# UMEssen/Body-and-Organ-Analysis

Hardware: AMD Instinct MI355X
Metric: CT volumes/sec (512^3 @1.5 mm, total+bca) on MI355X (higher is better)
Workload: dtype f16

## Files before the change

### body-and-organ-analysis_amd/csrc/ccl_bits.hip

```cpp
#include <string.h>

#include <algorithm>

#include "common.h"
#include "ccl_tile.h"

#define CB_CAP 1024
#define CB_BG 0xFFFFu

struct CbGeom {
    int Z, Y, X, W;
    int tx, ty, tz;
    size_t words;
    size_t vox;
    size_t tiles;
};

__host__ __device__ __forceinline__ unsigned cb_valid_word(int X, int w) {
    const int left = X - 32 * w;
    return left >= 32 ? 0xFFFFFFFFu : (left <= 0 ? 0u : ((1u << left) - 1u));
}

struct CbLut {
    unsigned char v[256];
};

__global__ __launch_bounds__(256) void k_bits_select(const unsigned char* __restrict__ seg, CbGeom g, CbLut lut, int n_masks, unsigned* __restrict__ bits) {
    __shared__ unsigned char s_lut[256];
    s_lut[threadIdx.x] = lut.v[threadIdx.x];
    __syncthreads();
    const size_t wi = (size_t)blockIdx.x * 256 + threadIdx.x;
    if (wi >= g.words) return;
    const int w = (int)(wi % g.W);
    const size_t row = wi / g.W;
    const unsigned char* p = seg + row * g.X + (size_t)w * 32;
    const int cnt = min(32, g.X - w * 32);
    unsigned out[8] = {0, 0, 0, 0, 0, 0, 0, 0};
    if (cnt == 32 && (((uintptr_t)p) & 15) == 0) {
        const uint4 a = *(const uint4*)p, b = *(const uint4*)(p + 16);
        const unsigned ww[8] = {a.x, a.y, a.z, a.w, b.x, b.y, b.z, b.w};
#pragma unroll
        for (int k = 0; k < 8; ++k)
#pragma unroll
            for (int j = 0; j < 4; ++j) {
                const unsigned m = s_lut[(ww[k] >> (8 * j)) & 0xFFu];
#pragma unroll
                for (int q = 0; q < 8; ++q) out[q] |= ((m >> q) & 1u) << (4 * k + j);
            }
    } else {
        for (int i = 0; i < cnt; ++i) {
            const unsigned m = s_lut[p[i]];
#pragma unroll
            for (int q = 0; q < 8; ++q) out[q] |= ((m >> q) & 1u) << i;
        }
    }
#pragma unroll
    for (int q = 0; q < 8; ++q)
        if (q < n_masks) bits[(size_t)q * g.words + wi] = out[q];
}

__global__ __launch_bounds__(256) void k_bits_unpack(const unsigned* __restrict__ bits, CbGeom g, unsigned char* __restrict__ out) {
    const size_t wi = (size_t)blockIdx.x * 256 + threadIdx.x;
    if (wi >= g.words) return;
    const int w = (int)(wi % g.W);
    const size_t row = wi / g.W;
    const unsigned v = bits[wi];
    unsigned char* p = out + row * g.X + (size_t)w * 32;
    const int cnt = min(32, g.X - w * 32);
    if (cnt == 32 && (((uintptr_t)p) & 15) == 0) {
        unsigned ww[8];
#pragma unroll
        for (int k = 0; k < 8; ++k) {
            const unsigned n4 = (v >> (4 * k)) & 0xfu;
            ww[k] = (n4 & 1u) | ((n4 & 2u) << 7) | ((n4 & 4u) << 14) | ((n4 & 8u) << 21);
        }
        *(uint4*)p = make_uint4(ww[0], ww[1], ww[2], ww[3]);
        *(uint4*)(p + 16) = make_uint4(ww[4], ww[5], ww[6], ww[7]);
    } else {
        for (int i = 0; i < cnt; ++i) p[i] = (unsigned char)((v >> i) & 1u);
    }
}

__global__ __launch_bounds__(256) void k_bits_erode_axis(const unsigned* __restrict__ in, CbGeom g, int axis, int lo, int hi, unsigned* __restrict__ out) {
    const size_t wi = (size_t)blockIdx.x * 256 + threadIdx.x;
    if (wi >= g.words) return;
    const int w = (int)(wi % g.W);
    const size_t row = wi / g.W;
    const int y = (int)(row % g.Y), z = (int)(row / g.Y);
    unsigned r = 0xFFFFFFFFu;
    if (axis == 2) {
        auto word = [&](int ww) -> unsigned {
            if (ww < 0 || ww >= g.W) return 0xFFFFFFFFu;
            return in[row * g.W + ww] | ~cb_valid_word(g.X, ww);
        };
        const unsigned prev = word(w - 1), cur = word(w), next = word(w + 1);
        for (int d = lo; d <= hi; ++d) {
            unsigned v;
            if (d == 0)
                v = cur;
            else if (d < 0)
                v = (cur << (-d)) | (prev >> (32 + d));
            else
                v = (cur >> d) | (next << (32 - d));
            r &= v;
        }
    } else {
        const int pos = axis == 0 ? z : y, len = axis == 0 ? g.Z : g.Y;
        const long long st = axis == 0 ? (long long)g.Y * g.W : (long long)g.W;
        for (int d = lo; d <= hi; ++d) {
            const int q = pos + d;
            if (q < 0 || q >= len) continue;
            r &= in[(long long)wi + d * st];
        }
    }
    out[wi] = r & cb_valid_word(g.X, w);
}

struct CbLabels {
    unsigned char v[8];
};
__global__ __launch_bounds__(256) void k_bits_assign(const unsigned* __restrict__ bits, CbGeom g, int n_masks, CbLabels labels, unsigned char* __restrict__ out) {
    const size_t wi = (size_t)blockIdx.x * 256 + threadIdx.x;
    if (wi >= g.words) return;
    const int w = (int)(wi % g.W);
    const size_t row = wi / g.W;
    unsigned m[8];
#pragma unroll
    for (int q = 0; q < 8; ++q) m[q] = q < n_masks ? bits[(size_t)q * g.words + wi] : 0u;
    unsigned char* p = out + row * g.X + (size_t)w * 32;
    const int cnt = min(32, g.X - w * 32);
    unsigned any = 0;
#pragma unroll
    for (int q = 0; q < 8; ++q) any |= m[q];
    if (!any) return;
    unsigned char b[32];
#pragma unroll
    for (int i = 0; i < 32; ++i) {
        unsigned char v = 0;
#pragma unroll
        for (int q = 0; q < 8; ++q)
            if ((m[q] >> i) & 1u) v = labels.v[q];
        b[i] = v;
    }
    if (cnt == 32 && (((uintptr_t)p) & 15) == 0) {
        const uint4 o0 = *(const uint4*)p, o1 = *(const uint4*)(p + 16);
        const unsigned oo[8] = {o0.x, o0.y, o0.z, o0.w, o1.x, o1.y, o1.z, o1.w};
        unsigned ww[8];
#pragma unroll
        for (int k = 0; k < 8; ++k) {
            unsigned v = 0;
#pragma unroll
            for (int j = 0; j < 4; ++j) {
                const unsigned keep = (oo[k] >> (8 * j)) & 0xFFu;
                v |= (((any >> (4 * k + j)) & 1u) ? (unsigned)b[4 * k + j] : keep) << (8 * j);
            }
            ww[k] = v;
        }
        *(uint4*)p = make_uint4(ww[0], ww[1], ww[2], ww[3]);
        *(uint4*)(p + 16) = make_uint4(ww[4], ww[5], ww[6], ww[7]);
    } else {
        for (int i = 0; i < cnt; ++i)
            if ((any >> i) & 1u) p[i] = b[i];
    }
}

__host__ __device__ inline int cb_fill_stride(int W) { return W | 1; }

__global__ __launch_bounds__(256) void k_bits_fill2d(const unsigned* __restrict__ in, CbGeom g, unsigned* __restrict__ out) {
    extern __shared__ unsigned int fsm2[];
    const int Y = g.Y, W = g.W, X = g.X;
    const int WP = cb_fill_stride(W);
    unsigned int* bg = fsm2;
    unsigned int* rc = fsm2 + (size_t)Y * WP;
    __shared__ int changed;
    const int tid = threadIdx.x;
    const size_t base = (size_t)blockIdx.y * g.words + (size_t)blockIdx.x * Y * W;
    const int nw = Y * W;
    for (int idx = tid; idx < nw; idx += 256) {
        const int y = idx / W, w = idx - y * W;
        const unsigned b = ~in[base + idx] & cb_valid_word(X, w);
        unsigned r = 0;
        if (y == 0 || y == Y - 1) r = b;
        if (w == 0) r |= b & 1u;
        if (w == W - 1) r |= b & (1u << ((X - 1) & 31));
        bg[y * WP + w] = b;
        rc[y * WP + w] = r;
    }
    __syncthreads();
    for (;;) {
        if (tid == 0) changed = 0;
        __syncthreads();
        int ch = 0;
        for (int y = tid; y < Y; y += 256) {
            unsigned int* rr = rc + y * WP;
            const unsigned int* bb = bg + y * WP;
            unsigned int carry = 0;
            for (int w = 0; w < W; ++w) {
                const unsigned int b = bb[w];
                unsigned int sd = rr[w] | (carry ? (b & 1u) : 0u);
                const unsigned long long sum = (unsigned long long)b + sd;
                const unsigned int nr = sd | ((b ^ (unsigned int)sum) & b);
                carry = (unsigned int)(sum >> 32);
                if (nr != rr[w]) { rr[w] = nr; ch = 1; }
            }
            carry = 0;
            for (int w = W - 1; w >= 0; --w) {
                const unsigned int b = __brev(bb[w]);
                unsigned int sd = __brev(rr[w]) | (carry ? (b & 1u) : 0u);
                const unsigned long long sum = (unsigned long long)b + sd;
                const unsigned int nr = __brev(sd | ((b ^ (unsigned int)sum) & b));
                carry = (unsigned int)(sum >> 32);
                if (nr != rr[w]) { rr[w] = nr; ch = 1; }
            }
        }
        __syncthreads();
        for (int idx = tid; idx < nw; idx += 256) {
            const int y = idx / W, li = idx + y * (WP - W);
            const unsigned int r = rc[li];
            const unsigned int up = y > 0 ? rc[li - WP] : 0u, dn = y < Y - 1 ? rc[li + WP] : 0u;
            const unsigned int nr = r | ((up | dn) & bg[li]);
            if (nr != r) { rc[li] = nr; ch = 1; }
        }
        if (ch) changed = 1;
        __syncthreads();
        if (!changed) break;
        __syncthreads();
    }
    for (int idx = tid; idx < nw; idx += 256) {
        const int y = idx / W, w = idx - y * W, li = y * WP + w;
        out[base + idx] = (~bg[li] | (bg[li] & ~rc[li])) & cb_valid_word(X, w);
    }
}

struct CbTab {
    int* parent;
    unsigned* size;
    int* first;
    int* ncomp;
    unsigned short* ids;
};

__device__ __forceinline__ unsigned cb_word(const unsigned* __restrict__ bits, const CbGeom& g, int m, int z, int y, int w, int inv) {
    if (z < 0 || y < 0 || w < 0 || z >= g.Z || y >= g.Y || w >= g.W) return 0u;
    const unsigned v = bits[(size_t)m * g.words + ((size_t)z * g.Y + y) * g.W + w];
    return inv ? (~v & cb_valid_word(g.X, w)) : v;
}

__global__ __launch_bounds__(256) void k_cb_local(const unsigned* __restrict__ bits, CbGeom g, int inv, CbTab T) {
    __shared__ int lab[CCL_TILE];
    __shared__ unsigned int rowbits[CCL_TY * CCL_TZ];
    __shared__ unsigned int rootbits[CCL_TY * CCL_TZ];
    __shared__ int rowpre[CCL_TY * CCL_TZ + 1];
    const int tid = threadIdx.x, m = blockIdx.y;
    int t = blockIdx.x;
    const int tx = t % g.tx;
    t /= g.tx;
    const int ty = t % g.ty, tz = t / g.ty;
    const int x0 = tx * CCL_TX, y0 = ty * CCL_TY, z0 = tz * CCL_TZ;
    const size_t tile = (size_t)m * g.tiles + blockIdx.x;
    {
        const int ly = tid % CCL_TY, lz = tid / CCL_TY;
        rowbits[tid] = cb_word(bits, g, m, z0 + lz, y0 + ly, tx, inv);
    }
    __syncthreads();
    {
        const unsigned w = rowbits[tid];
        const int all0 = __syncthreads_and(w == 0u);
        const int all1 = __syncthreads_and(w == 0xffffffffu);
        if (all0) {
            if (tid == 0) T.ncomp[tile] = 0;
            return;
        }
        if (all1) {
            if (tid == 0) {
                const int gid = (int)(blockIdx.x) * CB_CAP;
                const size_t e = (size_t)m * g.tiles * CB_CAP + gid;
                T.ncomp[tile] = -1;
                T.parent[e] = gid;
                T.size[e] = CCL_TILE;
                T.first[e] = (int)(((size_t)z0 * g.Y + y0) * g.X + x0);
            }
            return;
        }
    }
    ccl_tile_init_runs(rowbits, lab, tid);
    __syncthreads();
    ccl_tile_union_rows(rowbits, lab, tid);
    __syncthreads();
    int myroot[CCL_TILE / 256];
    ccl_tile_roots(rowbits, lab, tid, myroot);
    __syncthreads();
#pragma unroll
    for (int k = 0; k < CCL_TILE / 256; ++k) {
        const int r2 = (tid >> 5) + 8 * k, lx = tid & 31;
        const unsigned long long b = __ballot(myroot[k] == r2 * CCL_TX + lx);
        if (lx == 0) rootbits[r2] = (unsigned int)(b >> (32 * ((tid >> 5) & 1)));
    }
    unsigned int* cnt = (unsigned int*)lab;
#pragma unroll
    for (int k = 0; k < CCL_TILE / 256; ++k) cnt[tid + 256 * k] = 0;
    __syncthreads();
    {
        const int c = __popc(rootbits[tid]);
        int s = c;
#pragma unroll
        for (int d = 1; d < 64; d <<= 1) {
            const int o = __shfl_up(s, d);
            if ((tid & 63) >= d) s += o;
        }
        __shared__ int wtot[4];
        if ((tid & 63) == 63) wtot[tid >> 6] = s;
        __syncthreads();
        int basew = 0;
        for (int w = 0; w < (tid >> 6); ++w) basew += wtot[w];
        rowpre[tid] = basew + s - c;
        if (tid == 255) rowpre[256] = basew + s;
    }
    ccl_tile_count_runs(cnt, tid, myroot);
    __syncthreads();
    const int n_local = rowpre[256];
    int did[CCL_TILE / 256];
#pragma unroll
    for (int k = 0; k < CCL_TILE / 256; ++k) {
        const int r2 = (tid >> 5) + 8 * k, lx = tid & 31;
        did[k] = -1;
        if (myroot[k] == r2 * CCL_TX + lx) {
            const int d = rowpre[r2] + __popc(rootbits[r2] & ((1u << lx) - 1u));
            did[k] = d;
            const int gid = (int)blockIdx.x * CB_CAP + d;
            const size_t e = (size_t)m * g.tiles * CB_CAP + gid;
            const int ly = r2 % CCL_TY, lz = r2 / CCL_TY;
            T.parent[e] = gid;
            T.size[e] = cnt[r2 * CCL_TX + lx];
            T.first[e] = (int)(((size_t)(z0 + lz) * g.Y + (y0 + ly)) * g.X + (x0 + lx));
        }
    }
    __syncthreads();
#pragma unroll
    for (int k = 0; k < CCL_TILE / 256; ++k)
        if (did[k] >= 0) lab[((tid >> 5) + 8 * k) * CCL_TX + (tid & 31)] = did[k];
    if (tid == 0) T.ncomp[tile] = n_local;
    __syncthreads();
#pragma unroll
    for (int k = 0; k < CCL_TILE / 256; ++k) {
        const int r2 = (tid >> 5) + 8 * k, lx = tid & 31, ly = r2 % CCL_TY, lz = r2 / CCL_TY;
        const int x = x0 + lx, y = y0 + ly, z = z0 + lz;
        if (x >= g.X || y >= g.Y || z >= g.Z) continue;
        T.ids[(size_t)m * g.vox + ((size_t)z * g.Y + y) * g.X + x] = myroot[k] >= 0 ? (unsigned short)lab[myroot[k]] : (unsigned short)CB_BG;
    }
}

__device__ __forceinline__ int cb_gid(const CbGeom& g, const CbTab& T, int m, int x, int y, int z) {
    const int tile = ((z / CCL_TZ) * g.ty + (y / CCL_TY)) * g.tx + (x / CCL_TX);
    const int nc = T.ncomp[(size_t)m * g.tiles + tile];
    if (nc < 0) return tile * CB_CAP;
    return tile * CB_CAP + (int)T.ids[(size_t)m * g.vox + ((size_t)z * g.Y + y) * g.X + x];
}

__device__ __forceinline__ void cb_border_voxel(const unsigned* __restrict__ bits, const CbGeom& g, const CbTab& T, int m, int inv, int x, int y, int z) {
    const int lx = x % CCL_TX, ly = y % CCL_TY, lz = z % CCL_TZ;
    const int w = x >> 5;
    const unsigned me = cb_word(bits, g, m, z, y, w, inv);
    if (!((me >> lx) & 1u)) return;
    int* P = T.parent + (size_t)m * g.tiles * CB_CAP;
    int my = -1;
    auto mine = [&]() {
        if (my < 0) my = cb_gid(g, T, m, x, y, z);
        return my;
    };
    const bool me_full = T.ncomp[(size_t)m * g.tiles + ((z / CCL_TZ) * g.ty + (y / CCL_TY)) * g.tx + (x / CCL_TX)] < 0;
    auto link = [&](int xx, int yy, int zz) {
        if (me_full && T.ncomp[(size_t)m * g.tiles + ((zz / CCL_TZ) * g.ty + (yy / CCL_TY)) * g.tx + (xx / CCL_TX)] < 0) return;
        uf_union(P, mine(), cb_gid(g, T, m, xx, yy, zz));
    };
    auto row3 = [&](int yy, int zz, bool& b0, bool& b1, bool& b2) {
        const unsigned wc = cb_word(bits, g, m, zz, yy, w, inv);
        b1 = (wc >> lx) & 1u;
        b0 = lx > 0 ? ((wc >> (lx - 1)) & 1u) : (x > 0 && (cb_word(bits, g, m, zz, yy, w - 1, inv) >> 31));
        b2 = lx < 31 ? ((wc >> (lx + 1)) & 1u) : (x + 1 < g.X && (cb_word(bits, g, m, zz, yy, w + 1, inv) & 1u));
        if (x + 1 >= g.X) b2 = false;
    };
    bool own0, own1, own2;
    row3(y, z, own0, own1, own2);
    if (lx == CCL_TX - 1 && own2) link(x + 1, y, z);
    const bool left = own0;
#pragma unroll
    for (int r = 0; r < 4; ++r) {
        const int dz = r == 0 ? 0 : 1, dy = r == 0 ? 1 : r - 2;
        const int zz = z + dz, yy = y + dy;
        if (zz >= g.Z || yy < 0 || yy >= g.Y) continue;
        const bool row_other = (dz && lz == CCL_TZ - 1) || (dy == 1 && ly == CCL_TY - 1) || (dy == -1 && ly == 0);
        if (!row_other && lx != 0 && lx != CCL_TX - 1) continue;
        bool m0, m1, m2;
        row3(yy, zz, m0, m1, m2);
        if (row_other) {
            if (!left) {
                if (m1) {
                    link(x, yy, zz);
                } else {
                    if (m0) link(x - 1, yy, zz);
                    if (m2) link(x + 1, yy, zz);
                }
            } else if (m2 && !m1) {
                link(x + 1, yy, zz);
            }
        } else if (!m1) {
            if (m0 && lx == 0) link(x - 1, yy, zz);
            if (m2 && lx == CCL_TX - 1) link(x + 1, yy, zz);
        }
    }
}

__global__ __launch_bounds__(256) void k_cb_border_tiles(const unsigned* __restrict__ bits, CbGeom g, int inv, CbTab T) {
    const int m = blockIdx.y, tid = threadIdx.x;
    int t = blockIdx.x;
    const int tx = t % g.tx;
    t /= g.tx;
    const int ty = t % g.ty, tz = t / g.ty;
    const int nc = T.ncomp[(size_t)m * g.tiles + blockIdx.x];
    if (nc == 0) return;
    if (nc < 0) {
        int mixed = 0;
        if (tid < 13) {
            const int k = tid + 14;
            const int dx = k % 3 - 1, dy = (k / 3) % 3 - 1, dz = k / 9 - 1;
            const int nx = tx + dx, ny = ty + dy, nz = tz + dz;
            if (nx >= 0 && nx < g.tx && ny >= 0 && ny < g.ty && nz < g.tz) {
                const int nt = (nz * g.ty + ny) * g.tx + nx;
                const int nn = T.ncomp[(size_t)m * g.tiles + nt];
                if (nn < 0)
                    uf_union(T.parent + (size_t)m * g.tiles * CB_CAP, (int)blockIdx.x * CB_CAP, nt * CB_CAP);
                else if (nn > 0)
                    mixed = 1;
            }
        }
        if (!__syncthreads_or(mixed)) return;
    }
    const int x0 = tx * CCL_TX, y0 = ty * CCL_TY, z0 = tz * CCL_TZ;
    constexpr int N0 = CCL_TX * CCL_TY, N1 = 2 * (CCL_TZ - 1) * CCL_TX, N2 = 2 * (CCL_TY - 2) * (CCL_TZ - 1);
    for (int i = tid; i < N0 + N1 + N2; i += 256) {
        int lx, ly, lz;
        if (i < N0) {
            lx = i % CCL_TX; ly = i / CCL_TX; lz = CCL_TZ - 1;
        } else if (i < N0 + N1) {
            const int j = i - N0;
            lx = j % CCL_TX; lz = (j / CCL_TX) % (CCL_TZ - 1); ly = (j / (CCL_TX * (CCL_TZ - 1))) ? CCL_TY - 1 : 0;
        } else {
            const int j = i - N0 - N1;
            lx = (j & 1) ? CCL_TX - 1 : 0; ly = 1 + (j >> 1) % (CCL_TY - 2); lz = (j >> 1) / (CCL_TY - 2);
        }
        const int x = x0 + lx, y = y0 + ly, z = z0 + lz;
        if (x >= g.X || y >= g.Y || z >= g.Z) continue;
        cb_border_voxel(bits, g, T, m, inv, x, y, z);
    }
}

__global__ __launch_bounds__(256) void k_cb_resolve(CbGeom g, CbTab T, int n_masks) {
    const size_t wv = ((size_t)blockIdx.x * 256 + threadIdx.x) >> 6;
    const int lane = threadIdx.x & 63;
    if (wv >= g.tiles * (size_t)n_masks) return;
    const int m = (int)(wv / g.tiles), tile = (int)(wv % g.tiles);
    int nc = T.ncomp[wv];
    if (nc == 0) return;
    if (nc < 0) nc = 1;
    int* P = T.parent + (size_t)m * g.tiles * CB_CAP;
    unsigned* S = T.size + (size_t)m * g.tiles * CB_CAP;
    int* F = T.first + (size_t)m * g.tiles * CB_CAP;
    for (int k0 = 0; k0 < nc; k0 += 64) {
        const int k = k0 + lane;
        unsigned pend_c = 0u;
        int pend_root = 0, pend_first = 0;
        if (k < nc) {
            const int gid = tile * CB_CAP + k;
            int root = gid, p = AGENT_LOAD(&P[root]);
            while (p != root) {
                root = p;
                p = AGENT_LOAD(&P[root]);
            }
            if (root != gid) {
                __hip_atomic_store(&P[gid], root, __ATOMIC_RELAXED, __HIP_MEMORY_SCOPE_AGENT);
                pend_c = S[gid];
                pend_first = F[gid];
                pend_root = root;
            }
        }
#pragma unroll 1
        for (int round = 0; round < 3; ++round) {
            const unsigned long long act = __ballot(pend_c != 0u);
            if (!act) break;
            const int leader = __ffsll((long long)act) - 1;
            const int r0 = __shfl(pend_root, leader);
            const bool mine = pend_c != 0u && pend_root == r0;
            unsigned sum = mine ? pend_c : 0u;
            int fmin = mine ? pend_first : 0x7fffffff;
#pragma unroll
            for (int mm = 32; mm >= 1; mm >>= 1) {
                sum += __shfl_xor(sum, mm);
                fmin = min(fmin, __shfl_xor(fmin, mm));
            }
            if (lane == leader) {
                atomicAdd(&S[r0], sum);
                atomicMin(&F[r0], fmin);
            }
            if (mine) pend_c = 0u;
        }
        if (pend_c) {
            atomicAdd(&S[pend_root], pend_c);
            atomicMin(&F[pend_root], pend_first);
        }
    }
}

__global__ __launch_bounds__(256) void k_cb_remove_small(unsigned* __restrict__ bits, CbGeom g, int inv, CbTab T, unsigned max_size) {
    const size_t wi = (size_t)blockIdx.x * 256 + threadIdx.x;
    const int m = blockIdx.y;
    if (wi >= g.words) return;
    const int w = (int)(wi % g.W);
    const size_t row = wi / g.W;
    const int y = (int)(row % g.Y), z = (int)(row / g.Y);
    const unsigned orig = bits[(size_t)m * g.words + wi];
    const unsigned cur = inv ? (~orig & cb_valid_word(g.X, w)) : orig;
    if (!cur) return;
    const int tile = ((z / CCL_TZ) * g.ty + (y / CCL_TY)) * g.tx + w;
    const int nc = T.ncomp[(size_t)m * g.tiles + tile];
    const int* P = T.parent + (size_t)m * g.tiles * CB_CAP;
    const unsigned* S = T.size + (size_t)m * g.tiles * CB_CAP;
    unsigned small = 0;
    if (nc < 0) {
        const int gid = tile * CB_CAP;
        if (S[P[gid]] <= max_size) small = cur;
    } else {
        const unsigned short* idr = T.ids + (size_t)m * g.vox + row * g.X + (size_t)w * 32;
        unsigned rest = cur;
        int last_id = -1;
        bool last_small = false;
        while (rest) {
            const int i = __ffs((int)rest) - 1;
            rest &= rest - 1;
            const int id = idr[i];
            if (id != last_id) {
                last_id = id;
                last_small = S[P[tile * CB_CAP + id]] <= max_size;
            }
            if (last_small) small |= 1u << i;
        }
    }
    if (small) bits[(size_t)m * g.words + wi] = inv ? (orig | small) : (orig & ~small);
}

__global__ __launch_bounds__(256) void k_cb_best(CbGeom g, CbTab T, unsigned long long* best) {
    const size_t wv = ((size_t)blockIdx.x * 256 + threadIdx.x) >> 6;
    const int lane = threadIdx.x & 63;
    unsigned long long key = 0;
    if (wv < g.tiles) {
        int nc = T.ncomp[wv];
        if (nc < 0) nc = 1;
        const int tile = (int)wv;
        for (int k = lane; k < nc; k += 64) {
            const int gid = tile * CB_CAP + k;
            if (T.parent[gid] == gid) {
                const unsigned long long kk = ((unsigned long long)T.size[gid] << 32) | (unsigned long long)(0xFFFFFFFFu - (unsigned)T.first[gid]);
                key = kk > key ? kk : key;
            }
        }
    }
#pragma unroll
    for (int mm = 32; mm >= 1; mm >>= 1) {
        const unsigned long long o = __shfl_xor(key, mm);
        key = o > key ? o : key;
    }
    if (lane == 0 && key) atomicMax(best, key);
}

__global__ __launch_bounds__(256) void k_cb_apply_largest(const unsigned* __restrict__ bits, CbGeom g, CbTab T, const unsigned long long* best,
                                                          unsigned char* __restrict__ seg, int fill) {
    const size_t wi = (size_t)blockIdx.x * 256 + threadIdx.x;
    if (wi >= g.words) return;
    const unsigned cur = bits[wi];
    if (!cur) return;
    const unsigned long long b = *best;
    if (!b) return;
    const int best_first = (int)(0xFFFFFFFFu - (unsigned)(b & 0xFFFFFFFFull));
    const int w = (int)(wi % g.W);
    const size_t row = wi / g.W;
    const int y = (int)(row % g.Y), z = (int)(row / g.Y);
    const int tile = ((z / CCL_TZ) * g.ty + (y / CCL_TY)) * g.tx + w;
    const int nc = T.ncomp[tile];
    unsigned kill = 0;
    if (nc < 0) {
        if (T.first[T.parent[tile * CB_CAP]] != best_first) kill = cur;
    } else {
        const unsigned short* idr = T.ids + row * g.X + (size_t)w * 32;
        unsigned rest = cur;
        int last_id = -1;
        bool last_kill = false;
        while (rest) {
            const int i = __ffs((int)rest) - 1;
            rest &= rest - 1;
            const int id = idr[i];
            if (id != last_id) {
                last_id = id;
                last_kill = T.first[T.parent[tile * CB_CAP + id]] != best_first;
            }
            if (last_kill) kill |= 1u << i;
        }
    }
    unsigned char* p = seg + row * g.X + (size_t)w * 32;
    while (kill) {
        const int i = __ffs((int)kill) - 1;
        kill &= kill - 1;
        p[i] = (unsigned char)fill;
    }
}

static CbGeom cb_geom(int Z, int Y, int X) {
    CbGeom g;
    g.Z = Z; g.Y = Y; g.X = X;
    g.W = (X + 31) / 32;
    g.tx = g.W;
    g.ty = (Y + CCL_TY - 1) / CCL_TY;
    g.tz = (Z + CCL_TZ - 1) / CCL_TZ;
    g.words = (size_t)Z * Y * g.W;
    g.vox = (size_t)Z * Y * X;
    g.tiles = (size_t)g.tx * g.ty * g.tz;
    return g;
}

extern "C" size_t boa_bits_words(int Z, int Y, int X) { return (Z > 0 && Y > 0 && X > 0) ? cb_geom(Z, Y, X).words : 0; }

extern "C" int boa_bits_select(boa_ctx* c, const uint8_t* dev_seg, int Z, int Y, int X, const uint8_t host_lut[256], int n_masks, uint32_t* dev_bits) {
    BOA_REQUIRE(c && dev_seg && host_lut && dev_bits && Z > 0 && Y > 0 && X > 0 && n_masks >= 1 && n_masks <= 8, "boa_bits_select: bad argument");
    const CbGeom g = cb_geom(Z, Y, X);
    CbLut lut;
    memcpy(lut.v, host_lut, 256);
    KernelTimer t(c, BOA_K_MORPH, 0, (double)g.vox + 4.0 * (double)g.words * n_masks);
    hipLaunchKernelGGL(k_bits_select, dim3((unsigned)((g.words + 255) / 256)), dim3(256), 0, c->stream, dev_seg, g, lut, n_masks, dev_bits);
    t.stop();
    BOA_HIP_TRY(hipGetLastError());
    return BOA_OK;
}

extern "C" int boa_bits_unpack(boa_ctx* c, const uint32_t* dev_bits, int Z, int Y, int X, uint8_t* dev_out) {
    BOA_REQUIRE(c && dev_bits && dev_out && Z > 0 && Y > 0 && X > 0, "boa_bits_unpack: bad argument");
    const CbGeom g = cb_geom(Z, Y, X);
    KernelTimer t(c, BOA_K_MORPH, 0, (double)g.vox + 4.0 * (double)g.words);
    hipLaunchKernelGGL(k_bits_unpack, dim3((unsigned)((g.words + 255) / 256)), dim3(256), 0, c->stream, dev_bits, g, dev_out);
    t.stop();
    BOA_HIP_TRY(hipGetLastError());
    return BOA_OK;
}

extern "C" int boa_bits_assign_labels(boa_ctx* c, const uint32_t* dev_bits, int Z, int Y, int X, int n_masks, const uint8_t* host_labels, uint8_t* dev_out) {
    BOA_REQUIRE(c && dev_bits && host_labels && dev_out && Z > 0 && Y > 0 && X > 0 && n_masks >= 1 && n_masks <= 8, "boa_bits_assign_labels: bad argument");
    const CbGeom g = cb_geom(Z, Y, X);
    CbLabels lb;
    for (int q = 0; q < 8; ++q) lb.v[q] = q < n_masks ? host_labels[q] : 0;
    KernelTimer t(c, BOA_K_MORPH, 0, (double)g.vox + 4.0 * (double)g.words * n_masks);
    hipLaunchKernelGGL(k_bits_assign, dim3((unsigned)((g.words + 255) / 256)), dim3(256), 0, c->stream, dev_bits, g, n_masks, lb, dev_out);
    t.stop();
    BOA_HIP_TRY(hipGetLastError());
    return BOA_OK;
}

extern "C" int boa_bits_erode_u8(boa_ctx* c, const uint8_t* dev_mask, uint8_t* dev_out, int Z, int Y, int X, int lo, int hi) {
    BOA_REQUIRE(c && dev_mask && dev_out && Z > 0 && Y > 0 && X > 0 && lo <= 0 && hi >= 0 && lo > -32 && hi < 32, "boa_bits_erode_u8: bad argument");
    const CbGeom g = cb_geom(Z, Y, X);
    unsigned* a = nullptr;
    unsigned* b = nullptr;
    BOA_TRY(boa_malloc(c, g.words * 4, (void**)&a));
    if (int rc = boa_malloc(c, g.words * 4, (void**)&b)) {
        boa_free(c, a);
        return rc;
    }
    CbLut lut;
    lut.v[0] = 0;
    for (int i = 1; i < 256; ++i) lut.v[i] = 1;
    const unsigned grid = (unsigned)((g.words + 255) / 256);
    KernelTimer t(c, BOA_K_AGG, 0, 2.0 * (double)g.vox);
    hipLaunchKernelGGL(k_bits_select, dim3(grid), dim3(256), 0, c->stream, dev_mask, g, lut, 1, a);
    hipLaunchKernelGGL(k_bits_erode_axis, dim3(grid), dim3(256), 0, c->stream, a, g, 2, lo, hi, b);
    hipLaunchKernelGGL(k_bits_erode_axis, dim3(grid), dim3(256), 0, c->stream, b, g, 1, lo, hi, a);
    hipLaunchKernelGGL(k_bits_erode_axis, dim3(grid), dim3(256), 0, c->stream, a, g, 0, lo, hi, b);
    hipLaunchKernelGGL(k_bits_unpack, dim3(grid), dim3(256), 0, c->stream, b, g, dev_out);
    t.stop();
    const hipError_t e = hipGetLastError();
    boa_free(c, a);
    boa_free(c, b);
    BOA_HIP_TRY(e);
    return BOA_OK;
}

static size_t cb_lds_limit() {
    static const size_t lim = [] {
        int dev = 0, v = 0;
        if (hipGetDevice(&dev) == hipSuccess && hipDeviceGetAttribute(&v, hipDeviceAttributeSharedMemPerBlockOptin, dev) == hipSuccess && v > 0)
            return (size_t)std::min(v, 160 * 1024) - 10 * 1024;
        (void)hipGetLastError();
        return (size_t)150 * 1024;
    }();
    return lim;
}
extern "C" int boa_bits_fill_supported(int Y, int X) { return (size_t)Y * cb_fill_stride((X + 31) / 32) * 8 <= cb_lds_limit() ? 1 : 0; }

extern "C" int boa_bits_fill_holes_2d(boa_ctx* c, const uint32_t* dev_in, int Z, int Y, int X, int n_masks, uint32_t* dev_out) {
    BOA_REQUIRE(c && dev_in && dev_out && Z > 0 && Y > 0 && X > 0 && n_masks >= 1, "boa_bits_fill_holes_2d: bad argument");
    BOA_REQUIRE(boa_bits_fill_supported(Y, X), "boa_bits_fill_holes_2d: a %d x %d slice does not fit the LDS flood", Y, X);
    const CbGeom g = cb_geom(Z, Y, X);
    static bool once = (hipFuncSetAttribute((const void*)k_bits_fill2d, hipFuncAttributeMaxDynamicSharedMemorySize, 160 * 1024 - 256), true);
    (void)once;
    KernelTimer t(c, BOA_K_MORPH, 0, 8.0 * (double)g.words * n_masks);
    hipLaunchKernelGGL(k_bits_fill2d, dim3((unsigned)Z, (unsigned)n_masks), dim3(256), (size_t)Y * cb_fill_stride(g.W) * 8, c->stream, dev_in, g, dev_out);
    t.stop();
    BOA_HIP_TRY(hipGetLastError());
    return BOA_OK;
}

struct CbScratch {
    boa_ctx* c = nullptr;
    CbTab T{};
    int alloc(boa_ctx* ctx, const CbGeom& g, int n_masks) {
        c = ctx;
        const size_t ent = (size_t)n_masks * g.tiles * CB_CAP;
        BOA_TRY(boa_malloc(c, ent * sizeof(int), (void**)&T.parent));
        BOA_TRY(boa_malloc(c, ent * sizeof(unsigned), (void**)&T.size));
        BOA_TRY(boa_malloc(c, ent * sizeof(int), (void**)&T.first));
        BOA_TRY(boa_malloc(c, (size_t)n_masks * g.tiles * sizeof(int), (void**)&T.ncomp));
        BOA_TRY(boa_malloc(c, (size_t)n_masks * g.vox * sizeof(unsigned short), (void**)&T.ids));
        return BOA_OK;
    }
    ~CbScratch() {
        if (!c) return;
        if (T.parent) boa_free(c, T.parent);
        if (T.size) boa_free(c, T.size);
        if (T.first) boa_free(c, T.first);
        if (T.ncomp) boa_free(c, T.ncomp);
        if (T.ids) boa_free(c, T.ids);
    }
};

static void cb_label(boa_ctx* c, const uint32_t* bits, const CbGeom& g, int n_masks, int inv, const CbTab& T) {
    hipLaunchKernelGGL(k_cb_local, dim3((unsigned)g.tiles, (unsigned)n_masks), dim3(256), 0, c->stream, bits, g, inv, T);
    hipLaunchKernelGGL(k_cb_border_tiles, dim3((unsigned)g.tiles, (unsigned)n_masks), dim3(256), 0, c->stream, bits, g, inv, T);
    const size_t waves = g.tiles * (size_t)n_masks;
    hipLaunchKernelGGL(k_cb_resolve, dim3((unsigned)((waves * 64 + 255) / 256)), dim3(256), 0, c->stream, g, T, n_masks);
}

extern "C" int boa_bits_remove_small(boa_ctx* c, uint32_t* dev_bits, int Z, int Y, int X, int n_masks, uint32_t max_size, int invert) {
    BOA_REQUIRE(c && dev_bits && Z > 0 && Y > 0 && X > 0 && n_masks >= 1 && n_masks <= 64, "boa_bits_remove_small: bad argument");
    const CbGeom g = cb_geom(Z, Y, X);
    BOA_REQUIRE(g.vox < (1ull << 31) && g.tiles * CB_CAP < (1ull << 31), "boa_bits_remove_small: volume too large for int32 indices");
    CbScratch s;
    BOA_TRY(s.alloc(c, g, n_masks));
    KernelTimer t(c, BOA_K_MORPH, 0, (double)n_masks * (8.0 * (double)g.words + 4.0 * (double)g.vox));
    cb_label(c, dev_bits, g, n_masks, invert ? 1 : 0, s.T);
    hipLaunchKernelGGL(k_cb_remove_small, dim3((unsigned)((g.words + 255) / 256), (unsigned)n_masks), dim3(256), 0, c->stream, dev_bits, g, invert ? 1 : 0, s.T, max_size);
    t.stop();
    BOA_HIP_TRY(hipGetLastError());
    return BOA_OK;
}

extern "C" int boa_bits_filter_largest(boa_ctx* c, const uint32_t* dev_bits, int Z, int Y, int X, uint8_t* dev_seg, int fill_value) {
    BOA_REQUIRE(c && dev_bits && dev_seg && Z > 0 && Y > 0 && X > 0, "boa_bits_filter_largest: bad argument");
    const CbGeom g = cb_geom(Z, Y, X);
    BOA_REQUIRE(g.vox < (1ull << 31) && g.tiles * CB_CAP < (1ull << 31), "boa_bits_filter_largest: volume too large for int32 indices");
    CbScratch s;
    BOA_TRY(s.alloc(c, g, 1));
    unsigned long long* d_best = nullptr;
    BOA_TRY(boa_malloc(c, sizeof(unsigned long long), (void**)&d_best));
    hipError_t e0 = hipMemsetAsync(d_best, 0, sizeof(unsigned long long), c->stream);
    if (e0 != hipSuccess) {
        boa_free(c, d_best);
        BOA_HIP_TRY(e0);
    }
    KernelTimer t(c, BOA_K_MORPH, 0, 8.0 * (double)g.words + 5.0 * (double)g.vox);
    cb_label(c, dev_bits, g, 1, 0, s.T);
    hipLaunchKernelGGL(k_cb_best, dim3((unsigned)((g.tiles * 64 + 255) / 256)), dim3(256), 0, c->stream, g, s.T, d_best);
    hipLaunchKernelGGL(k_cb_apply_largest, dim3((unsigned)((g.words + 255) / 256)), dim3(256), 0, c->stream, dev_bits, g, s.T, d_best, dev_seg, fill_value);
    t.stop();
    const hipError_t e = hipGetLastError();
    boa_free(c, d_best);
    BOA_HIP_TRY(e);
    return BOA_OK;
}
```

### body-and-organ-analysis_amd/csrc/ccl_tile.h

```cpp
#pragma once
#include <hip/hip_runtime.h>

#define AGENT_LOAD(p) __hip_atomic_load((p), __ATOMIC_RELAXED, __HIP_MEMORY_SCOPE_AGENT)

template <bool HALVE = true>
__device__ __forceinline__ int uf_find(int* L, int i) {
    int p = AGENT_LOAD(&L[i]);
    while (p != i) {
        const int gp = AGENT_LOAD(&L[p]);
        if (HALVE && gp != p) __hip_atomic_store(&L[i], gp, __ATOMIC_RELAXED, __HIP_MEMORY_SCOPE_AGENT);
        i = p;
        p = gp;
    }
    return i;
}

template <bool HALVE = true>
__device__ __forceinline__ void uf_union(int* L, int a, int b) {
    while (true) {
        a = uf_find<HALVE>(L, a);
        b = uf_find<HALVE>(L, b);
        if (a == b) return;
        if (a < b) {
            const int t = a;
            a = b;
            b = t;
        }
        const int old = atomicMin(&L[a], b);
        if (old == a) return;
        a = old;
    }
}

__device__ __forceinline__ int lds_find(volatile int* L, int i) {
    int p = L[i];
    while (p != i) {
        const int gp = L[p];
        if (gp != p) L[i] = gp;
        i = p;
        p = gp;
    }
    return i;
}

__device__ __forceinline__ void lds_union(int* L, int a, int b) {
    while (true) {
        a = lds_find(L, a);
        b = lds_find(L, b);
        if (a == b) return;
        if (a < b) {
            const int t = a;
            a = b;
            b = t;
        }
        const int old = atomicMin(&L[a], b);
        if (old == a) return;
        a = old;
    }
}

#define CCL_TX 32
#define CCL_TY 16
#define CCL_TZ 16
#define CCL_TILE (CCL_TX * CCL_TY * CCL_TZ)


__device__ __forceinline__ void ccl_tile_init_runs(const unsigned int* rowbits, int* lab, int tid) {
    for (int r2 = tid >> 5; r2 < CCL_TY * CCL_TZ; r2 += 8) {
        const int lx = tid & 31;
        const unsigned int me = rowbits[r2];
        const unsigned int starts = me & ~(me << 1);
        const unsigned int upto = starts & (0xffffffffu >> (31 - lx));
        lab[r2 * CCL_TX + lx] = ((me >> lx) & 1u) ? r2 * CCL_TX + (31 - __clz((int)upto)) : -1;
    }
}

__device__ __forceinline__ void ccl_tile_union_rows(const unsigned int* rowbits, int* lab, int tid) {
    for (int r2 = tid >> 5; r2 < CCL_TY * CCL_TZ; r2 += 8) {
        const int lx = tid & 31, ly = r2 % CCL_TY, lz = r2 / CCL_TY;
        const unsigned int me = rowbits[r2];
        if (!((me >> lx) & 1u)) continue;
        const int i = r2 * CCL_TX + lx;
        const bool a_l = lx > 0 && ((me >> (lx - 1)) & 1u), a_r = lx + 1 < CCL_TX && ((me >> (lx + 1)) & 1u);
#pragma unroll
        for (int r = 0; r < 4; ++r) {
            const int dz = r == 0 ? 0 : 1, dy = r == 0 ? 1 : r - 2;
            const int zz = lz + dz, yy = ly + dy;
            if (zz >= CCL_TZ || yy < 0 || yy >= CCL_TY) continue;
            const int rr = zz * CCL_TY + yy;
            const unsigned int w = rowbits[rr];
            const bool m0 = lx > 0 && ((w >> (lx - 1)) & 1u), m1 = (w >> lx) & 1u, m2 = lx + 1 < CCL_TX && ((w >> (lx + 1)) & 1u);
            const int row = rr * CCL_TX;
            if (m1) {
                if (!(a_l && m0)) lds_union(lab, i, row + lx);
            } else {
                if (m2 && !a_r) lds_union(lab, i, row + lx + 1);
                if (m0 && !a_l) lds_union(lab, i, row + lx - 1);
            }
        }
    }
}

__device__ __forceinline__ void ccl_tile_roots(const unsigned int* rowbits, int* lab, int tid, int (&myroot)[CCL_TILE / 256]) {
#pragma unroll
    for (int k = 0; k < CCL_TILE / 256; ++k) {
        const int r2 = (tid >> 5) + 8 * k, lx = tid & 31;
        myroot[k] = -1;
        if ((rowbits[r2] >> lx) & 1u) myroot[k] = lds_find(lab, r2 * CCL_TX + lx);
    }
}

__device__ __forceinline__ void ccl_tile_count_runs(unsigned int* cnt, int tid, const int (&myroot)[CCL_TILE / 256]) {
#pragma unroll
    for (int k = 0; k < CCL_TILE / 256; ++k) {
        const int lx = tid & 31;
        const int prev = __shfl_up(myroot[k], 1);
        const bool lead = lx == 0 || prev != myroot[k];
        const unsigned int leads = (unsigned int)(__ballot(lead) >> (32 * ((tid >> 5) & 1)));
        if (lead && myroot[k] >= 0) {
            const unsigned int after = lx == 31 ? 0u : (leads >> (lx + 1));
            const int len = after ? __ffs((int)after) : 32 - lx;
            atomicAdd(&cnt[myroot[k]], (unsigned int)len);
        }
    }
}
```

Before: 0.5970.

## Replace 2D hole-fill flood with run-based union-find and batch tile row unions

```diff
diff --git a/body-and-organ-analysis_amd/csrc/ccl_bits.hip b/body-and-organ-analysis_amd/csrc/ccl_bits.hip
--- a/body-and-organ-analysis_amd/csrc/ccl_bits.hip
+++ b/body-and-organ-analysis_amd/csrc/ccl_bits.hip
@@ -166,8 +166,49 @@
 
 __host__ __device__ inline int cb_fill_stride(int W) { return W | 1; }
 
-__global__ __launch_bounds__(256) void k_bits_fill2d(const unsigned* __restrict__ in, CbGeom g, unsigned* __restrict__ out) {
-    extern __shared__ unsigned int fsm2[];
+__device__ __forceinline__ unsigned f2_find(volatile unsigned short* L, unsigned i) {
+    unsigned p = L[i];
+    while (p != i) {
+        const unsigned gp = L[p];
+        if (gp != p) L[i] = (unsigned short)gp;
+        i = p;
+        p = gp;
+    }
+    return i;
+}
+
+__device__ __forceinline__ unsigned f2_atomic_min(unsigned short* L, unsigned a, unsigned b) {
+    unsigned* wp = (unsigned*)L + (a >> 1);
+    const int sh = (int)(a & 1u) * 16;
+    unsigned old = *(volatile unsigned*)wp;
+    while (true) {
+        const unsigned cur = (old >> sh) & 0xFFFFu;
+        if (cur <= b) return cur;
+        const unsigned prev = atomicCAS(wp, old, (old & ~(0xFFFFu << sh)) | (b << sh));
+        if (prev == old) return cur;
+        old = prev;
+    }
+}
+
+__device__ __forceinline__ void f2_union(unsigned short* L, unsigned a, unsigned b) {
+    while (true) {
+        a = f2_find(L, a);
+        b = f2_find(L, b);
+        if (a == b) return;
+        if (a < b) {
+            const unsigned t = a;
+            a = b;
+            b = t;
+        }
+        const unsigned old = f2_atomic_min(L, a, b);
+        if (old == a) return;
+        a = old;
+    }
+}
+
+#define FILL_NT 1024
+
+__device__ void cb_fill_flood(const unsigned* __restrict__ in, const CbGeom& g, unsigned* __restrict__ out, unsigned int* fsm2) {
     const int Y = g.Y, W = g.W, X = g.X;
     const int WP = cb_fill_stride(W);
     unsigned int* bg = fsm2;
@@ -176,7 +217,7 @@
     const int tid = threadIdx.x;
     const size_t base = (size_t)blockIdx.y * g.words + (size_t)blockIdx.x * Y * W;
     const int nw = Y * W;
-    for (int idx = tid; idx < nw; idx += 256) {
+    for (int idx = tid; idx < nw; idx += FILL_NT) {
         const int y = idx / W, w = idx - y * W;
         const unsigned b = ~in[base + idx] & cb_valid_word(X, w);
         unsigned r = 0;
@@ -191,7 +232,7 @@
         if (tid == 0) changed = 0;
         __syncthreads();
         int ch = 0;
-        for (int y = tid; y < Y; y += 256) {
+        for (int y = tid; y < Y; y += FILL_NT) {
             unsigned int* rr = rc + y * WP;
             const unsigned int* bb = bg + y * WP;
             unsigned int carry = 0;
@@ -214,7 +255,7 @@
             }
         }
         __syncthreads();
-        for (int idx = tid; idx < nw; idx += 256) {
+        for (int idx = tid; idx < nw; idx += FILL_NT) {
             const int y = idx / W, li = idx + y * (WP - W);
             const unsigned int r = rc[li];
             const unsigned int up = y > 0 ? rc[li - WP] : 0u, dn = y < Y - 1 ? rc[li + WP] : 0u;
@@ -226,10 +267,148 @@
         if (!changed) break;
         __syncthreads();
     }
-    for (int idx = tid; idx < nw; idx += 256) {
+    for (int idx = tid; idx < nw; idx += FILL_NT) {
         const int y = idx / W, w = idx - y * W, li = y * WP + w;
         out[base + idx] = (~bg[li] | (bg[li] & ~rc[li])) & cb_valid_word(X, w);
     }
+}
+
+__host__ __device__ inline unsigned cb_fill_par_offset(int nw) { return ((unsigned)nw * 6u + 3u) & ~3u; }
+
+__global__ __launch_bounds__(FILL_NT) void k_bits_fill2d(const unsigned* __restrict__ in, CbGeom g, unsigned cap, unsigned* __restrict__ out) {
+    extern __shared__ unsigned int fsm2[];
+    if (cap == 0u) {
+        cb_fill_flood(in, g, out, fsm2);
+        return;
+    }
+    __shared__ int wtot[FILL_NT / 64];
+    __shared__ int s_y1, s_again;
+    const int Y = g.Y, W = g.W, X = g.X, nw = Y * W, tid = threadIdx.x;
+    const size_t base = (size_t)blockIdx.y * g.words + (size_t)blockIdx.x * Y * W;
+    unsigned int* U = fsm2;
+    unsigned short* rb = (unsigned short*)(fsm2 + nw);
+    unsigned short* par = (unsigned short*)((char*)fsm2 + cb_fill_par_offset(nw));
+    unsigned* R = out + base;
+    const int max_runs = (int)cap - 1;
+    for (int idx = tid; idx < nw; idx += FILL_NT) U[idx] = ~in[base + idx] & cb_valid_word(X, idx % W);
+    __syncthreads();
+    for (int idx = tid; idx < nw; idx += FILL_NT) R[idx] = 0u;
+    auto starts = [&](int idx, int w) -> unsigned {
+        const unsigned b = U[idx];
+        return b & ~((b << 1) | (w > 0 ? U[idx - 1] >> 31 : 0u));
+    };
+    auto run_of = [&](unsigned id0, unsigned st, int x) -> unsigned { return id0 + __popc(st & (0xFFFFFFFFu >> (31 - x))) - 1u; };
+    const int chunk = ((nw + FILL_NT - 1) / FILL_NT) | 1;
+    const int i0 = min(nw, tid * chunk), i1 = min(nw, i0 + chunk);
+    bool have_r = false;
+    for (int sweep = 0, max_sweeps = nw * 16 + 1; sweep < max_sweeps; ++sweep) {
+        if (tid == 0) s_again = 0;
+        for (int y0 = 0, y1 = 0; y0 < Y; y0 = y1) {
+            if (tid == 0) s_y1 = y0;
+            const int f0 = max(i0, y0 * W);
+            int c = 0;
+            for (int idx = f0, w = f0 % W; idx < i1; ++idx) {
+                c += __popc(starts(idx, w));
+                if (++w == W) w = 0;
+            }
+            int sc = c;
+#pragma unroll
+            for (int d = 1; d < 64; d <<= 1) {
+                const int o = __shfl_up(sc, d);
+                if ((tid & 63) >= d) sc += o;
+            }
+            if ((tid & 63) == 63) wtot[tid >> 6] = sc;
+            __syncthreads();
+            int first = sc - c, total = 0;
+            for (int k = 0; k < FILL_NT / 64; ++k) {
+                if (k < (tid >> 6)) first += wtot[k];
+                total += wtot[k];
+            }
+            if (total <= max_runs) {
+                if (tid == 0) s_y1 = Y;
+            } else {
+                int run = first;
+                for (int idx = f0, w = f0 % W; idx < i1; ++idx) {
+                    if (w == 0 && run <= max_runs) atomicMax(&s_y1, idx / W);
+                    run += __popc(starts(idx, w));
+                    if (++w == W) w = 0;
+                }
+            }
+            __syncthreads();
+            y1 = s_y1;
+            if (y1 <= y0) y1 = y0 + 1;
+            const int e1 = min(i1, y1 * W);
+            {
+                int run = first + 1;
+                for (int idx = f0, w = f0 % W; idx < e1; ++idx) {
+                    rb[idx] = (unsigned short)run;
+                    run += __popc(starts(idx, w));
+                    if (++w == W) w = 0;
+                }
+            }
+            __syncthreads();
+            if (tid == 0) par[0] = 0;
+            for (int idx = y0 * W + tid; idx < y1 * W; idx += FILL_NT) {
+                const int y = idx / W, w = idx - y * W;
+                const unsigned st = starts(idx, w);
+                const int k = __popc(st);
+                const unsigned id0 = rb[idx];
+                const bool edge_row = y == 0 || y == Y - 1;
+                for (int j = 0; j < k; ++j) par[id0 + j] = (edge_row || (j == 0 && w == 0 && (st & 1u))) ? (unsigned short)0 : (unsigned short)(id0 + j);
+            }
+            __syncthreads();
+            for (int idx = y0 * W + tid; idx < y1 * W; idx += FILL_NT) {
+                const int y = idx / W, w = idx - y * W;
+                const unsigned b = U[idx];
+                if (!b) continue;
+                const unsigned st = starts(idx, w), id0 = rb[idx];
+                if (w == W - 1 && ((b >> ((X - 1) & 31)) & 1u)) f2_union(par, run_of(id0, st, (X - 1) & 31), 0u);
+                if (have_r) {
+                    unsigned sd = b & ((y > 0 ? R[idx - W] : 0u) | (y < Y - 1 ? R[idx + W] : 0u));
+                    while (sd) {
+                        const int x = __ffs((int)sd) - 1;
+                        f2_union(par, run_of(id0, st, x), 0u);
+                        sd &= ~(b & ~(b + (1u << x)));
+                    }
+                }
+                if (y >= y1 - 1) continue;
+                const unsigned o = b & U[idx + W];
+                if (!o) continue;
+                unsigned os = o & ~((o << 1) | (w > 0 ? (U[idx - 1] & U[idx + W - 1]) >> 31 : 0u));
+                const unsigned st_dn = starts(idx + W, w), id0_dn = rb[idx + W];
+                while (os) {
+                    const int x = __ffs((int)os) - 1;
+                    os &= os - 1;
+                    f2_union(par, run_of(id0, st, x), run_of(id0_dn, st_dn, x));
+                }
+            }
+            __syncthreads();
+            for (int idx = y0 * W + tid; idx < y1 * W; idx += FILL_NT) {
+                const int w = idx % W;
+                const unsigned b = U[idx];
+                const unsigned st = starts(idx, w), id0 = rb[idx];
+                unsigned rest = b, reach = 0;
+                while (rest) {
+                    const int x = __ffs((int)rest) - 1;
+                    const unsigned rm = rest & ~(rest + (1u << x));
+                    if (f2_find(par, run_of(id0, st, x)) == 0u) reach |= rm;
+                    rest &= ~rm;
+                }
+                if (reach) {
+                    R[idx] |= reach;
+                    if (idx < (y0 + 1) * W && y0 > 0 && (reach & U[idx - W])) s_again = 1;
+                }
+            }
+            __syncthreads();
+            for (int idx = y0 * W + tid; idx < y1 * W; idx += FILL_NT) U[idx] &= ~R[idx];
+            have_r = true;
+            __syncthreads();
+        }
+        const int again = s_again;
+        __syncthreads();
+        if (!again) break;
+    }
+    for (int idx = tid; idx < nw; idx += FILL_NT) R[idx] = cb_valid_word(X, idx % W) & ~R[idx];
 }
 
 struct CbTab {
@@ -357,7 +536,8 @@
     return tile * CB_CAP + (int)T.ids[(size_t)m * g.vox + ((size_t)z * g.Y + y) * g.X + x];
 }
 
-__device__ __forceinline__ void cb_border_voxel(const unsigned* __restrict__ bits, const CbGeom& g, const CbTab& T, int m, int inv, int x, int y, int z) {
+__device__ __forceinline__ void cb_border_voxel(const unsigned* __restrict__ bits, const CbGeom& g, const CbTab& T, int m, int inv, int x, int y, int z,
+                                                int nc, int (&memo)[2]) {
     const int lx = x % CCL_TX, ly = y % CCL_TY, lz = z % CCL_TZ;
     const int w = x >> 5;
     const unsigned me = cb_word(bits, g, m, z, y, w, inv);
@@ -365,13 +545,20 @@
     int* P = T.parent + (size_t)m * g.tiles * CB_CAP;
     int my = -1;
     auto mine = [&]() {
-        if (my < 0) my = cb_gid(g, T, m, x, y, z);
+        if (my < 0) {
+            const int tile = ((z / CCL_TZ) * g.ty + (y / CCL_TY)) * g.tx + (x / CCL_TX);
+            my = nc < 0 ? tile * CB_CAP : tile * CB_CAP + (int)T.ids[(size_t)m * g.vox + ((size_t)z * g.Y + y) * g.X + x];
+        }
         return my;
     };
-    const bool me_full = T.ncomp[(size_t)m * g.tiles + ((z / CCL_TZ) * g.ty + (y / CCL_TY)) * g.tx + (x / CCL_TX)] < 0;
+    const bool me_full = nc < 0;
     auto link = [&](int xx, int yy, int zz) {
         if (me_full && T.ncomp[(size_t)m * g.tiles + ((zz / CCL_TZ) * g.ty + (yy / CCL_TY)) * g.tx + (xx / CCL_TX)] < 0) return;
-        uf_union(P, mine(), cb_gid(g, T, m, xx, yy, zz));
+        const int a = mine(), b = cb_gid(g, T, m, xx, yy, zz);
+        if (a == memo[0] && b == memo[1]) return;
+        memo[0] = a;
+        memo[1] = b;
+        uf_union(P, a, b);
     };
     auto row3 = [&](int yy, int zz, bool& b0, bool& b1, bool& b2) {
         const unsigned wc = cb_word(bits, g, m, zz, yy, w, inv);
@@ -438,6 +625,7 @@
     }
     const int x0 = tx * CCL_TX, y0 = ty * CCL_TY, z0 = tz * CCL_TZ;
     constexpr int N0 = CCL_TX * CCL_TY, N1 = 2 * (CCL_TZ - 1) * CCL_TX, N2 = 2 * (CCL_TY - 2) * (CCL_TZ - 1);
+    int memo[2] = {-1, -1};
     for (int i = tid; i < N0 + N1 + N2; i += 256) {
         int lx, ly, lz;
         if (i < N0) {
@@ -451,7 +639,7 @@
         }
         const int x = x0 + lx, y = y0 + ly, z = z0 + lz;
         if (x >= g.X || y >= g.Y || z >= g.Z) continue;
-        cb_border_voxel(bits, g, T, m, inv, x, y, z);
+        cb_border_voxel(bits, g, T, m, inv, x, y, z, nc, memo);
     }
 }
 
@@ -700,6 +888,17 @@
     }();
     return lim;
 }
+static size_t cb_fill_lds_bytes(int Y, int X) {
+    const int W = (X + 31) / 32;
+    const size_t flood = (size_t)Y * cb_fill_stride(W) * 8;
+    const size_t max_runs = std::min((size_t)65534, (size_t)Y * ((X + 1) / 2));
+    const size_t labels = cb_fill_par_offset(Y * W) + 2 * (max_runs + 1);
+    return std::min(cb_lds_limit(), std::max(flood, labels));
+}
+static unsigned cb_fill_cap(int Y, int X, size_t lds) {
+    const size_t cap = std::min((size_t)65535, (lds - cb_fill_par_offset(Y * ((X + 31) / 32))) / 2);
+    return (size_t)(X + 1) / 2 + 1 <= cap ? (unsigned)cap : 0u;
+}
 extern "C" int boa_bits_fill_supported(int Y, int X) { return (size_t)Y * cb_fill_stride((X + 31) / 32) * 8 <= cb_lds_limit() ? 1 : 0; }
 
 extern "C" int boa_bits_fill_holes_2d(boa_ctx* c, const uint32_t* dev_in, int Z, int Y, int X, int n_masks, uint32_t* dev_out) {
@@ -708,8 +907,9 @@
     const CbGeom g = cb_geom(Z, Y, X);
     static bool once = (hipFuncSetAttribute((const void*)k_bits_fill2d, hipFuncAttributeMaxDynamicSharedMemorySize, 160 * 1024 - 256), true);
     (void)once;
+    const size_t lds = cb_fill_lds_bytes(Y, X);
     KernelTimer t(c, BOA_K_MORPH, 0, 8.0 * (double)g.words * n_masks);
-    hipLaunchKernelGGL(k_bits_fill2d, dim3((unsigned)Z, (unsigned)n_masks), dim3(256), (size_t)Y * cb_fill_stride(g.W) * 8, c->stream, dev_in, g, dev_out);
+    hipLaunchKernelGGL(k_bits_fill2d, dim3((unsigned)Z, (unsigned)n_masks), dim3(FILL_NT), lds, c->stream, dev_in, g, cb_fill_cap(Y, X, lds), dev_out);
     t.stop();
     BOA_HIP_TRY(hipGetLastError());
     return BOA_OK;
diff --git a/body-and-organ-analysis_amd/csrc/ccl_tile.h b/body-and-organ-analysis_amd/csrc/ccl_tile.h
--- a/body-and-organ-analysis_amd/csrc/ccl_tile.h
+++ b/body-and-organ-analysis_amd/csrc/ccl_tile.h
@@ -76,27 +76,26 @@
 }
 
 __device__ __forceinline__ void ccl_tile_union_rows(const unsigned int* rowbits, int* lab, int tid) {
-    for (int r2 = tid >> 5; r2 < CCL_TY * CCL_TZ; r2 += 8) {
-        const int lx = tid & 31, ly = r2 % CCL_TY, lz = r2 / CCL_TY;
-        const unsigned int me = rowbits[r2];
-        if (!((me >> lx) & 1u)) continue;
-        const int i = r2 * CCL_TX + lx;
-        const bool a_l = lx > 0 && ((me >> (lx - 1)) & 1u), a_r = lx + 1 < CCL_TX && ((me >> (lx + 1)) & 1u);
-#pragma unroll
-        for (int r = 0; r < 4; ++r) {
-            const int dz = r == 0 ? 0 : 1, dy = r == 0 ? 1 : r - 2;
-            const int zz = lz + dz, yy = ly + dy;
-            if (zz >= CCL_TZ || yy < 0 || yy >= CCL_TY) continue;
-            const int rr = zz * CCL_TY + yy;
-            const unsigned int w = rowbits[rr];
-            const bool m0 = lx > 0 && ((w >> (lx - 1)) & 1u), m1 = (w >> lx) & 1u, m2 = lx + 1 < CCL_TX && ((w >> (lx + 1)) & 1u);
-            const int row = rr * CCL_TX;
-            if (m1) {
-                if (!(a_l && m0)) lds_union(lab, i, row + lx);
-            } else {
-                if (m2 && !a_r) lds_union(lab, i, row + lx + 1);
-                if (m0 && !a_l) lds_union(lab, i, row + lx - 1);
-            }
+    constexpr int ROWS = CCL_TY * CCL_TZ;
+    for (int p = tid; p < 4 * ROWS; p += 256) {
+        const int r = p / ROWS, r2 = p % ROWS, ly = r2 % CCL_TY, lz = r2 / CCL_TY;
+        const int dz = r == 0 ? 0 : 1, dy = r == 0 ? 1 : r - 2;
+        const int zz = lz + dz, yy = ly + dy;
+        if (zz >= CCL_TZ || yy < 0 || yy >= CCL_TY) continue;
+        const int rr = zz * CCL_TY + yy;
+        const unsigned int me = rowbits[r2], w = rowbits[rr];
+        if (!me || !w) continue;
+        const unsigned int o = me & w, alone = me & ~w;
+        unsigned int s0 = o & ~(o << 1);
+        unsigned int s1 = alone & (w >> 1) & ~(me >> 1);
+        unsigned int s2 = alone & (w << 1) & ~(me << 1);
+        while (s0 | s1 | s2) {
+            const int d = s0 ? 0 : (s1 ? 1 : -1);
+            const unsigned int s = s0 ? s0 : (s1 ? s1 : s2);
+            const int lx = __ffs((int)s) - 1;
+            const unsigned int rest = s & (s - 1);
+            if (s0) s0 = rest; else if (s1) s1 = rest; else s2 = rest;
+            lds_union(lab, r2 * CCL_TX + lx, rr * CCL_TX + lx + d);
         }
     }
 }
```

After: 0.6026 (median of 6 runs). No clear change (+0.9%).
